# Frikallo/parakeet.cpp

Hardware: NVIDIA H100
Metric: audio-seconds/sec (RTFx) tdt-ctc-110m 10s clips (higher is better)
Workload: dtype bf16x3

## Files before the change

### parakeet.cpp_b200/csrc/attention_tc.cu

```cuda
#include "kernels.h"

namespace pk {
namespace {

constexpr int BQ = 64, BKV = 64;
constexpr int NPW = 128;
constexpr int LDG_ = 84;
constexpr int TCA_THREADS = 128;

template <int HD, bool QS>
struct __align__(16) AttnSmem {
    static constexpr int LDS_ = HD + 8;
    bf16 k_hi[BKV * LDS_], k_lo[BKV * LDS_];
    bf16 v_hi[BKV * LDS_], v_lo[BKV * LDS_];
    bf16 pp_hi[NPW * LDS_], pp_lo[NPW * LDS_];
    float g[QS ? 1 : 4][QS ? 4 : 16 * LDG_];
    bf16 q[QS ? 4 : 1][QS ? BQ * LDS_ : 8];
};
static_assert(sizeof(float) * 4 * 16 * LDG_ <= sizeof(bf16) * 2 * BKV * (128 + 8), "G patches must fit in the K tile");

__device__ __forceinline__ uint32_t smem_addr(const void *p) { return (uint32_t)__cvta_generic_to_shared(p); }
__device__ __forceinline__ void mma_bf16(float (&d)[4], const uint32_t (&a)[4], uint32_t b0, uint32_t b1) {
    asm volatile(
        "mma.sync.aligned.m16n8k16.row.col.f32.bf16.bf16.f32 {%0, %1, %2, %3}, {%4, %5, %6, %7}, {%8, %9}, {%0, %1, %2, %3};"
        : "+f"(d[0]), "+f"(d[1]), "+f"(d[2]), "+f"(d[3])
        : "r"(a[0]), "r"(a[1]), "r"(a[2]), "r"(a[3]), "r"(b0), "r"(b1));
}
__device__ __forceinline__ void ldsm_x4(uint32_t (&r)[4], uint32_t addr) {
    asm volatile("ldmatrix.sync.aligned.m8n8.x4.shared.b16 {%0, %1, %2, %3}, [%4];"
                 : "=r"(r[0]), "=r"(r[1]), "=r"(r[2]), "=r"(r[3]) : "r"(addr));
}
__device__ __forceinline__ void ldsm_x4_t(uint32_t (&r)[4], uint32_t addr) {
    asm volatile("ldmatrix.sync.aligned.m8n8.x4.trans.shared.b16 {%0, %1, %2, %3}, [%4];"
                 : "=r"(r[0]), "=r"(r[1]), "=r"(r[2]), "=r"(r[3]) : "r"(addr));
}
__device__ __forceinline__ void cp_async16(uint32_t dst, const void *src, int src_bytes) {
    asm volatile("cp.async.cg.shared.global [%0], [%1], 16, %2;" ::"r"(dst), "l"(src), "r"(src_bytes) : "memory");
}
__device__ __forceinline__ void split2(float x, float y, uint32_t &hi, uint32_t &lo) {
    __nv_bfloat162 h = __floats2bfloat162_rn(x, y);
    float2 hf = __bfloat1622float2(h);
    __nv_bfloat162 l = __floats2bfloat162_rn(x - hf.x, y - hf.y);
    hi = *reinterpret_cast<uint32_t *>(&h);
    lo = *reinterpret_cast<uint32_t *>(&l);
}
__device__ __forceinline__ float ex2_approx(float x) {
    float y;
    asm("ex2.approx.ftz.f32 %0, %1;" : "=f"(y) : "f"(x));
    return y;
}

template <int LDS_>
__device__ __forceinline__ uint32_t bfrag_addr(const bf16 *base, int n0, int k0, int lane) {
    return smem_addr(base + (n0 + ((lane >> 4) << 3) + (lane & 7)) * LDS_ + k0 + (((lane >> 3) & 1) << 3));
}
template <int LDS_>
__device__ __forceinline__ uint32_t afrag_addr(const bf16 *base, int m0, int k0, int lane) {
    return smem_addr(base + (m0 + (lane & 7) + (((lane >> 3) & 1) << 3)) * LDS_ + k0 + ((lane >> 4) << 3));
}
template <int LDS_>
__device__ __forceinline__ uint32_t bfrag_t_addr(const bf16 *base, int k0, int n0, int lane) {
    return smem_addr(base + (k0 + (((lane >> 3) & 1) << 3) + (lane & 7)) * LDS_ + n0 + ((lane >> 4) << 3));
}

template <int HD, bool QS>
__global__ void __launch_bounds__(TCA_THREADS, QS ? 1 : 2)
relpos_attention_tc_kernel(const float *__restrict__ q32, const float *__restrict__ pos_u, const float *__restrict__ pos_v,
                           const bf16 *__restrict__ qkv_hi, const bf16 *__restrict__ qkv_lo, int ld_qkv,
                           const int32_t *__restrict__ row_off, const bf16 *__restrict__ pp_hi,
                           const bf16 *__restrict__ pp_lo, int tmax, int d_model, ActBuf out) {
    pdl_wait();
    pdl_trigger();
    extern __shared__ __align__(16) uint8_t smraw[];
    using SM = AttnSmem<HD, QS>;
    constexpr int LDS_ = SM::LDS_, KS = HD / 16, NBO = HD / 8, CH = HD / 8;
    SM &sm = *reinterpret_cast<SM *>(smraw);
    const int b = blockIdx.z, h = blockIdx.y;
    const int r0 = row_off[b], T = row_off[b + 1] - r0;
    const int i0 = blockIdx.x * BQ;
    if (i0 >= T) return;
    const int tid = threadIdx.x, warp = tid >> 5, lane = tid & 31, g = lane >> 2, c = lane & 3;
    const int wrow = warp * 16;

    uint32_t qu_h[QS ? 1 : KS][4], qu_l[QS ? 1 : KS][4], qv_h[QS ? 1 : KS][4], qv_l[QS ? 1 : KS][4];
    constexpr int NQ = QS ? BQ * (HD / 4) / TCA_THREADS : 1;
    float4 qq[NQ];
    float2 qraw[QS ? 1 : KS][4];
    if (!QS) {
        const int ia = i0 + wrow + g, ib = ia + 8;
#pragma unroll
        for (int ks = 0; ks < (QS ? 1 : KS); ++ks)
#pragma unroll
            for (int e = 0; e < 4; ++e) {
                const int row = (e & 1) ? ib : ia;
                const int col = h * HD + ks * 16 + ((e >> 1) << 3) + 2 * c;
                qraw[ks][e] = make_float2(0.f, 0.f);
                if (row < T) qraw[ks][e] = *reinterpret_cast<const float2 *>(q32 + (size_t)(r0 + row) * d_model + col);
            }
    } else {
#pragma unroll
        for (int it = 0; it < NQ; ++it) {
            const int idx = tid + it * TCA_THREADS, i = idx / (HD / 4), c4 = (idx % (HD / 4)) * 4;
            qq[it] = make_float4(0.f, 0.f, 0.f, 0.f);
            if (i0 + i < T) qq[it] = *reinterpret_cast<const float4 *>(q32 + (size_t)(r0 + i0 + i) * d_model + h * HD + c4);
        }
    }

    float m_run[2] = {-INFINITY, -INFINITY}, l_run[2] = {0.f, 0.f};
    float oacc[NBO][4];
#pragma unroll
    for (int nb = 0; nb < NBO; ++nb)
#pragma unroll
        for (int e = 0; e < 4; ++e) oacc[nb][e] = 0.f;
    float *gs = QS ? reinterpret_cast<float *>(sm.k_hi) + warp * 16 * LDG_ : sm.g[QS ? 0 : warp];
    const uint32_t sk_hi = smem_addr(sm.k_hi), sk_lo = smem_addr(sm.k_lo), sv_hi = smem_addr(sm.v_hi), sv_lo = smem_addr(sm.v_lo);
    const uint32_t sp_hi = smem_addr(sm.pp_hi), sp_lo = smem_addr(sm.pp_lo);

    for (int j0 = 0; j0 < T; j0 += BKV) {
        __syncthreads();
        for (int idx = tid; idx < BKV * CH; idx += TCA_THREADS) {
            const int j = idx / CH, ch = idx % CH;
            const bool ok = (j0 + j < T);
            const size_t o = (size_t)(r0 + (ok ? j0 + j : 0)) * ld_qkv + h * HD + ch * 8;
            const uint32_t so = (uint32_t)(j * LDS_ + ch * 8) * 2u;
            const int nb = ok ? 16 : 0;
            cp_async16(sk_hi + so, qkv_hi + o, nb);
            cp_async16(sk_lo + so, qkv_lo + o, nb);
            cp_async16(sv_hi + so, qkv_hi + o + d_model, nb);
            cp_async16(sv_lo + so, qkv_lo + o + d_model, nb);
        }
        const int pmin = i0 - (j0 + BKV - 1);
        for (int idx = tid; idx < NPW * CH; idx += TCA_THREADS) {
            const int w = idx / CH, ch = idx % CH;
            const int prow = pmin + w + tmax - 1;
            const bool ok = (prow >= 0 && prow < 2 * tmax - 1);
            const size_t o = (size_t)(ok ? prow : 0) * d_model + h * HD + ch * 8;
            const uint32_t so = (uint32_t)(w * LDS_ + ch * 8) * 2u;
            const int nb = ok ? 16 : 0;
            cp_async16(sp_hi + so, pp_hi + o, nb);
            cp_async16(sp_lo + so, pp_lo + o, nb);
        }
        asm volatile("cp.async.commit_group;" ::: "memory");
        if (!QS && j0 == 0) {
            const int ia = i0 + wrow + g, ib = ia + 8;
#pragma unroll
            for (int ks = 0; ks < (QS ? 1 : KS); ++ks)
#pragma unroll
                for (int e = 0; e < 4; ++e) {
                    const int row = (e & 1) ? ib : ia;
                    const int col = h * HD + ks * 16 + ((e >> 1) << 3) + 2 * c;
                    const float2 bu = __ldg(reinterpret_cast<const float2 *>(pos_u + col)), bv = __ldg(reinterpret_cast<const float2 *>(pos_v + col));
                    const float2 qv2 = qraw[ks][e];
                    if (row < T) {
                        split2(qv2.x + bu.x, qv2.y + bu.y, qu_h[ks][e], qu_l[ks][e]);
                        split2(qv2.x + bv.x, qv2.y + bv.y, qv_h[ks][e], qv_l[ks][e]);
                    } else {
                        qu_h[ks][e] = qu_l[ks][e] = qv_h[ks][e] = qv_l[ks][e] = 0u;
                    }
                }
        }
        if (QS && j0 == 0) {
#pragma unroll
            for (int it = 0; it < NQ; ++it) {
                const int idx = tid + it * TCA_THREADS, i = idx / (HD / 4), c4 = (idx % (HD / 4)) * 4;
                const bool ok = (i0 + i < T);
                const float4 bu = __ldg(reinterpret_cast<const float4 *>(pos_u + h * HD + c4)), bv = __ldg(reinterpret_cast<const float4 *>(pos_v + h * HD + c4));
                uint2 uh = make_uint2(0u, 0u), ul = uh, vh = uh, vl = uh;
                if (ok) {
                    split2(qq[it].x + bu.x, qq[it].y + bu.y, uh.x, ul.x);
                    split2(qq[it].z + bu.z, qq[it].w + bu.w, uh.y, ul.y);
                    split2(qq[it].x + bv.x, qq[it].y + bv.y, vh.x, vl.x);
                    split2(qq[it].z + bv.z, qq[it].w + bv.w, vh.y, vl.y);
                }
                const int so = i * LDS_ + c4;
                *reinterpret_cast<uint2 *>(sm.q[0] + so) = uh;
                *reinterpret_cast<uint2 *>(sm.q[QS ? 1 : 0] + so) = ul;
                *reinterpret_cast<uint2 *>(sm.q[QS ? 2 : 0] + so) = vh;
                *reinterpret_cast<uint2 *>(sm.q[QS ? 3 : 0] + so) = vl;
            }
        }
        asm volatile("cp.async.wait_group 0;" ::: "memory");
        __syncthreads();

        float sacc[8][4];
#pragma unroll
        for (int nb = 0; nb < 8; ++nb)
#pragma unroll
            for (int e = 0; e < 4; ++e) sacc[nb][e] = 0.f;
#pragma unroll
        for (int ks = 0; ks < KS; ++ks) {
            uint32_t ah_[4], al_[4];
            if (QS) {
                ldsm_x4(ah_, afrag_addr<LDS_>(sm.q[0], wrow, ks * 16, lane));
                ldsm_x4(al_, afrag_addr<LDS_>(sm.q[QS ? 1 : 0], wrow, ks * 16, lane));
            }
            const uint32_t (&ah)[4] = QS ? ah_ : qu_h[QS ? 0 : ks];
            const uint32_t (&al)[4] = QS ? al_ : qu_l[QS ? 0 : ks];
#pragma unroll
            for (int np = 0; np < 4; ++np) {
                uint32_t bh[4], bl[4];
                ldsm_x4(bh, bfrag_addr<LDS_>(sm.k_hi, np * 16, ks * 16, lane));
                ldsm_x4(bl, bfrag_addr<LDS_>(sm.k_lo, np * 16, ks * 16, lane));
                mma_bf16(sacc[2 * np], ah, bh[0], bh[1]);
                mma_bf16(sacc[2 * np + 1], ah, bh[2], bh[3]);
                mma_bf16(sacc[2 * np], ah, bl[0], bl[1]);
                mma_bf16(sacc[2 * np + 1], ah, bl[2], bl[3]);
                mma_bf16(sacc[2 * np], al, bh[0], bh[1]);
                mma_bf16(sacc[2 * np + 1], al, bh[2], bh[3]);
            }
        }
        {
            float gacc[10][4];
#pragma unroll
            for (int nb = 0; nb < 10; ++nb)
#pragma unroll
                for (int e = 0; e < 4; ++e) gacc[nb][e] = 0.f;
#pragma unroll
            for (int ks = 0; ks < KS; ++ks) {
                uint32_t ah_[4], al_[4];
                if (QS) {
                    ldsm_x4(ah_, afrag_addr<LDS_>(sm.q[QS ? 2 : 0], wrow, ks * 16, lane));
                    ldsm_x4(al_, afrag_addr<LDS_>(sm.q[QS ? 3 : 0], wrow, ks * 16, lane));
                }
                const uint32_t (&ah)[4] = QS ? ah_ : qv_h[QS ? 0 : ks];
                const uint32_t (&al)[4] = QS ? al_ : qv_l[QS ? 0 : ks];
#pragma unroll
                for (int np = 0; np < 5; ++np) {
                    uint32_t bh[4], bl[4];
                    ldsm_x4(bh, bfrag_addr<LDS_>(sm.pp_hi, wrow + np * 16, ks * 16, lane));
                    ldsm_x4(bl, bfrag_addr<LDS_>(sm.pp_lo, wrow + np * 16, ks * 16, lane));
                    mma_bf16(gacc[2 * np], ah, bh[0], bh[1]);
                    mma_bf16(gacc[2 * np + 1], ah, bh[2], bh[3]);
                    mma_bf16(gacc[2 * np], ah, bl[0], bl[1]);
                    mma_bf16(gacc[2 * np + 1], ah, bl[2], bl[3]);
                    mma_bf16(gacc[2 * np], al, bh[0], bh[1]);
                    mma_bf16(gacc[2 * np + 1], al, bh[2], bh[3]);
                }
            }
            if (QS) __syncthreads();
#pragma unroll
            for (int nb = 0; nb < 10; ++nb) {
                *reinterpret_cast<float2 *>(gs + g * LDG_ + nb * 8 + 2 * c) = make_float2(gacc[nb][0], gacc[nb][1]);
                *reinterpret_cast<float2 *>(gs + (g + 8) * LDG_ + nb * 8 + 2 * c) = make_float2(gacc[nb][2], gacc[nb][3]);
            }
            __syncwarp();
#pragma unroll
            for (int nb = 0; nb < 8; ++nb)
#pragma unroll
                for (int e = 0; e < 2; ++e) {
                    const int jj = nb * 8 + 2 * c + e;
                    sacc[nb][e] += gs[g * LDG_ + g + (BKV - 1) - jj];
                    sacc[nb][2 + e] += gs[(g + 8) * LDG_ + g + 8 + (BKV - 1) - jj];
                }
            __syncwarp();
        }
        constexpr float kScale = (HD == 64 ? 0.125f : 0.08838834764831845f) * 1.4426950408889634f;
        static_assert(HD == 64 || HD == 128, "head_dim");
        float alpha[2];
#pragma unroll
        for (int hrow = 0; hrow < 2; ++hrow) {
            float mx = -INFINITY;
#pragma unroll
            for (int nb = 0; nb < 8; ++nb)
#pragma unroll
                for (int e = 0; e < 2; ++e) {
                    const int jj = nb * 8 + 2 * c + e;
                    float s = sacc[nb][hrow * 2 + e] * kScale;
                    s = (j0 + jj < T) ? s : -INFINITY;
                    sacc[nb][hrow * 2 + e] = s;
                    mx = fmaxf(mx, s);
                }
            mx = fmaxf(mx, __shfl_xor_sync(0xffffffffu, mx, 1));
            mx = fmaxf(mx, __shfl_xor_sync(0xffffffffu, mx, 2));
            const float m_new = fmaxf(m_run[hrow], mx);
            alpha[hrow] = ex2_approx(m_run[hrow] - m_new);
            float sum = 0.f;
#pragma unroll
            for (int nb = 0; nb < 8; ++nb)
#pragma unroll
                for (int e = 0; e < 2; ++e) {
                    const float pexp = ex2_approx(sacc[nb][hrow * 2 + e] - m_new);
                    sacc[nb][hrow * 2 + e] = pexp;
                    sum += pexp;
                }
            sum += __shfl_xor_sync(0xffffffffu, sum, 1);
            sum += __shfl_xor_sync(0xffffffffu, sum, 2);
            l_run[hrow] = l_run[hrow] * alpha[hrow] + sum;
            m_run[hrow] = m_new;
        }
#pragma unroll
        for (int nb = 0; nb < NBO; ++nb) {
            oacc[nb][0] *= alpha[0];
            oacc[nb][1] *= alpha[0];
            oacc[nb][2] *= alpha[1];
            oacc[nb][3] *= alpha[1];
        }
#pragma unroll
        for (int kk = 0; kk < BKV / 16; ++kk) {
            uint32_t ph[4], pl[4];
            split2(sacc[2 * kk][0], sacc[2 * kk][1], ph[0], pl[0]);
            split2(sacc[2 * kk][2], sacc[2 * kk][3], ph[1], pl[1]);
            split2(sacc[2 * kk + 1][0], sacc[2 * kk + 1][1], ph[2], pl[2]);
            split2(sacc[2 * kk + 1][2], sacc[2 * kk + 1][3], ph[3], pl[3]);
#pragma unroll
            for (int np = 0; np < HD / 16; ++np) {
                uint32_t bh[4], bl[4];
                ldsm_x4_t(bh, bfrag_t_addr<LDS_>(sm.v_hi, kk * 16, np * 16, lane));
                ldsm_x4_t(bl, bfrag_t_addr<LDS_>(sm.v_lo, kk * 16, np * 16, lane));
                mma_bf16(oacc[2 * np], ph, bh[0], bh[1]);
                mma_bf16(oacc[2 * np + 1], ph, bh[2], bh[3]);
                mma_bf16(oacc[2 * np], ph, bl[0], bl[1]);
                mma_bf16(oacc[2 * np + 1], ph, bl[2], bl[3]);
                mma_bf16(oacc[2 * np], pl, bh[0], bh[1]);
                mma_bf16(oacc[2 * np + 1], pl, bh[2], bh[3]);
            }
        }
    }
#pragma unroll
    for (int hrow = 0; hrow < 2; ++hrow) {
        const int i = i0 + wrow + g + hrow * 8;
        if (i >= T) continue;
        const float inv = 1.0f / l_run[hrow];
#pragma unroll
        for (int nb = 0; nb < NBO; ++nb) {
            const size_t idx = (size_t)(r0 + i) * d_model + h * HD + nb * 8 + 2 * c;
            const float x = oacc[nb][hrow * 2] * inv, y = oacc[nb][hrow * 2 + 1] * inv;
            if (out.f32) *reinterpret_cast<float2 *>(out.f32 + idx) = make_float2(x, y);
            if (out.hi) {
                uint32_t hi, lo;
                split2(x, y, hi, lo);
                *reinterpret_cast<uint32_t *>(out.hi + idx) = hi;
                if (out.lo) *reinterpret_cast<uint32_t *>(out.lo + idx) = lo;
            }
        }
    }
}

}

template <int HD, bool QS>
static bool launch_attn_t(const float *q32, const float *pos_u, const float *pos_v, const bf16 *qkv_hi, const bf16 *qkv_lo, int ld_qkv,
                          const int32_t *row_off, int n_utt, int max_T,
                          int n_heads, const bf16 *pp_hi, const bf16 *pp_lo, int tmax, int d_model, ActBuf out, cudaStream_t st) {
    using SM = AttnSmem<HD, QS>;
    static PerDeviceFlag attr_flag;
    bool &attr = attr_flag.cur();
    if (!attr) {
        if (cudaFuncSetAttribute(relpos_attention_tc_kernel<HD, QS>, cudaFuncAttributeMaxDynamicSharedMemorySize,
                                 (int)sizeof(SM)) != cudaSuccess)
            return false;
        attr = true;
    }
    dim3 grid((max_T + BQ - 1) / BQ, n_heads, n_utt);
    launch_pdl(relpos_attention_tc_kernel<HD, QS>, dim3(grid), dim3(TCA_THREADS), sizeof(SM), st, q32, pos_u, pos_v, qkv_hi, qkv_lo, ld_qkv, row_off, pp_hi, pp_lo,
                                                                              tmax, d_model, out);
    return true;
}

bool launch_relpos_attention_tc(const float *q32, const float *pos_u, const float *pos_v, const bf16 *qkv_hi, const bf16 *qkv_lo,
                                int ld_qkv, const int32_t *row_off, int n_utt, int max_T, int n_heads, int head_dim, const bf16 *pp_hi,
                                const bf16 *pp_lo, int tmax, int d_model, ActBuf out, cudaStream_t st) {
    if (!q32 || !pos_u || !pos_v || !qkv_hi || !qkv_lo || !pp_hi || !pp_lo) return false;
    if (head_dim == 64)
        return launch_attn_t<64, false>(q32, pos_u, pos_v, qkv_hi, qkv_lo, ld_qkv, row_off, n_utt, max_T, n_heads, pp_hi, pp_lo, tmax, d_model, out, st);
    if (head_dim == 128)
        return launch_attn_t<128, true>(q32, pos_u, pos_v, qkv_hi, qkv_lo, ld_qkv, row_off, n_utt, max_T, n_heads, pp_hi, pp_lo, tmax, d_model, out, st);
    return false;
}

}
```

Measured before the change: 44070.

## Make relpos attention persistent with double-buffered cp.async K/V/pos pipeline

Converts the relative-position attention kernel into a persistent grid that loops over (query block, head, utterance) items and prefetches the next item's data. K, V and positional tiles are staged through cp.async groups so loads overlap the QK, G and PV MMA stages. The positional window becomes a ring of 64-row slots reused across KV tiles instead of being reloaded as 128 rows each step. Q fragments are rebuilt from registers with the bias added on the fly, replacing the shared-memory Q staging. For head_dim 128 the block is now 8 warps with 128 query rows. This adds more synchronisation points and code complexity, and the persistent grid may balance poorly when there are few items.

```diff
diff --git a/parakeet.cpp_b200/csrc/attention_tc.cu b/parakeet.cpp_b200/csrc/attention_tc.cu
--- a/parakeet.cpp_b200/csrc/attention_tc.cu
+++ b/parakeet.cpp_b200/csrc/attention_tc.cu
@@ -3,21 +3,19 @@
 namespace pk {
 namespace {
 
-constexpr int BQ = 64, BKV = 64;
-constexpr int NPW = 128;
+constexpr int BKV = 64;
 constexpr int LDG_ = 84;
-constexpr int TCA_THREADS = 128;
-
-template <int HD, bool QS>
+
+template <int HD, int NW>
 struct __align__(16) AttnSmem {
-    static constexpr int LDS_ = HD + 8;
-    bf16 k_hi[BKV * LDS_], k_lo[BKV * LDS_];
-    bf16 v_hi[BKV * LDS_], v_lo[BKV * LDS_];
-    bf16 pp_hi[NPW * LDS_], pp_lo[NPW * LDS_];
-    float g[QS ? 1 : 4][QS ? 4 : 16 * LDG_];
-    bf16 q[QS ? 4 : 1][QS ? BQ * LDS_ : 8];
+    static constexpr int BQ = 16 * NW, NSLOT = NW / 4 + 1, LDS_ = HD + 8;
+    bf16 k[2][BKV * LDS_];
+    bf16 v[2][BKV * LDS_];
+    bf16 pp[NSLOT][2][BKV * LDS_];
+    float g[NW][16 * LDG_];
 };
-static_assert(sizeof(float) * 4 * 16 * LDG_ <= sizeof(bf16) * 2 * BKV * (128 + 8), "G patches must fit in the K tile");
+static_assert(sizeof(AttnSmem<128, 8>) <= 227 * 1024, "head_dim 128: one CTA per SM");
+static_assert(2 * (sizeof(AttnSmem<64, 4>) + 1024) <= 228 * 1024, "head_dim 64: two CTAs per SM");
 
 __device__ __forceinline__ uint32_t smem_addr(const void *p) { return (uint32_t)__cvta_generic_to_shared(p); }
 __device__ __forceinline__ void mma_bf16(float (&d)[4], const uint32_t (&a)[4], uint32_t b0, uint32_t b1) {
@@ -37,6 +35,8 @@
 __device__ __forceinline__ void cp_async16(uint32_t dst, const void *src, int src_bytes) {
     asm volatile("cp.async.cg.shared.global [%0], [%1], 16, %2;" ::"r"(dst), "l"(src), "r"(src_bytes) : "memory");
 }
+__device__ __forceinline__ void cp_async_commit() { asm volatile("cp.async.commit_group;" ::: "memory"); }
+__device__ __forceinline__ void cp_async_wait1() { asm volatile("cp.async.wait_group 1;" ::: "memory"); }
 __device__ __forceinline__ void split2(float x, float y, uint32_t &hi, uint32_t &lo) {
     __nv_bfloat162 h = __floats2bfloat162_rn(x, y);
     float2 hf = __bfloat1622float2(h);
@@ -51,199 +51,199 @@
 }
 
 template <int LDS_>
-__device__ __forceinline__ uint32_t bfrag_addr(const bf16 *base, int n0, int k0, int lane) {
-    return smem_addr(base + (n0 + ((lane >> 4) << 3) + (lane & 7)) * LDS_ + k0 + (((lane >> 3) & 1) << 3));
+__device__ __forceinline__ uint32_t bfrag_addr(uint32_t base, int n0, int k0, int lane) {
+    return base + 2u * (uint32_t)((n0 + ((lane >> 4) << 3) + (lane & 7)) * LDS_ + k0 + (((lane >> 3) & 1) << 3));
 }
 template <int LDS_>
-__device__ __forceinline__ uint32_t afrag_addr(const bf16 *base, int m0, int k0, int lane) {
-    return smem_addr(base + (m0 + (lane & 7) + (((lane >> 3) & 1) << 3)) * LDS_ + k0 + ((lane >> 4) << 3));
-}
-template <int LDS_>
-__device__ __forceinline__ uint32_t bfrag_t_addr(const bf16 *base, int k0, int n0, int lane) {
-    return smem_addr(base + (k0 + (((lane >> 3) & 1) << 3) + (lane & 7)) * LDS_ + n0 + ((lane >> 4) << 3));
-}
-
-template <int HD, bool QS>
-__global__ void __launch_bounds__(TCA_THREADS, QS ? 1 : 2)
+__device__ __forceinline__ uint32_t bfrag_t_addr(uint32_t base, int k0, int n0, int lane) {
+    return base + 2u * (uint32_t)((k0 + (((lane >> 3) & 1) << 3) + (lane & 7)) * LDS_ + n0 + ((lane >> 4) << 3));
+}
+
+template <int HD>
+__device__ __forceinline__ void qb_frag(const float2 (&q2)[4], const float *__restrict__ bias, int col0, bool oka, bool okb,
+                                        uint32_t (&hi)[4], uint32_t (&lo)[4]) {
+#pragma unroll
+    for (int e = 0; e < 4; ++e) {
+        const float2 bb = __ldg(reinterpret_cast<const float2 *>(bias + col0 + ((e >> 1) << 3)));
+        if ((e & 1) ? okb : oka) {
+            split2(q2[e].x + bb.x, q2[e].y + bb.y, hi[e], lo[e]);
+        } else {
+            hi[e] = lo[e] = 0u;
+        }
+    }
+}
+
+template <int HD, int NW>
+__global__ void __launch_bounds__(32 * NW, NW == 4 ? 2 : 1)
 relpos_attention_tc_kernel(const float *__restrict__ q32, const float *__restrict__ pos_u, const float *__restrict__ pos_v,
                            const bf16 *__restrict__ qkv_hi, const bf16 *__restrict__ qkv_lo, int ld_qkv,
                            const int32_t *__restrict__ row_off, const bf16 *__restrict__ pp_hi,
-                           const bf16 *__restrict__ pp_lo, int tmax, int d_model, ActBuf out) {
+                           const bf16 *__restrict__ pp_lo, int tmax, int d_model, int n_qb, int n_heads, int n_items, ActBuf out) {
     pdl_wait();
     pdl_trigger();
     extern __shared__ __align__(16) uint8_t smraw[];
-    using SM = AttnSmem<HD, QS>;
+    using SM = AttnSmem<HD, NW>;
+    constexpr int BQ = SM::BQ, NSLOT = SM::NSLOT, NTHR = 32 * NW;
     constexpr int LDS_ = SM::LDS_, KS = HD / 16, NBO = HD / 8, CH = HD / 8;
+    constexpr uint32_t PLANE = BKV * LDS_ * 2u;
     SM &sm = *reinterpret_cast<SM *>(smraw);
-    const int b = blockIdx.z, h = blockIdx.y;
-    const int r0 = row_off[b], T = row_off[b + 1] - r0;
-    const int i0 = blockIdx.x * BQ;
-    if (i0 >= T) return;
     const int tid = threadIdx.x, warp = tid >> 5, lane = tid & 31, g = lane >> 2, c = lane & 3;
     const int wrow = warp * 16;
-
-    uint32_t qu_h[QS ? 1 : KS][4], qu_l[QS ? 1 : KS][4], qv_h[QS ? 1 : KS][4], qv_l[QS ? 1 : KS][4];
-    constexpr int NQ = QS ? BQ * (HD / 4) / TCA_THREADS : 1;
-    float4 qq[NQ];
-    float2 qraw[QS ? 1 : KS][4];
-    if (!QS) {
-        const int ia = i0 + wrow + g, ib = ia + 8;
-#pragma unroll
-        for (int ks = 0; ks < (QS ? 1 : KS); ++ks)
+    const uint32_t sk = smem_addr(sm.k[0]), sv = smem_addr(sm.v[0]), sp = smem_addr(sm.pp[0][0]);
+
+    struct Item { int it, h, i0, r0, T; };
+    auto decode = [&](int it) {
+        Item x;
+        x.it = it;
+        x.i0 = (it % n_qb) * BQ;
+        x.h = (it / n_qb) % n_heads;
+        const int b = it / (n_qb * n_heads);
+        x.r0 = row_off[b];
+        x.T = row_off[b + 1] - x.r0;
+        return x;
+    };
+    auto next_item = [&](int it) {
+        for (; it < n_items; it += gridDim.x)
+            if (decode(it).i0 < decode(it).T) return it;
+        return n_items;
+    };
+    auto copy_kv = [&](uint32_t dst, const Item &x, int j0, int plane_off) {
+        for (int idx = tid; idx < BKV * CH; idx += NTHR) {
+            const int j = idx / CH, ch = idx % CH;
+            const bool ok = (j0 + j < x.T);
+            const size_t o = (size_t)(x.r0 + (ok ? j0 + j : 0)) * ld_qkv + plane_off + x.h * HD + ch * 8;
+            const uint32_t so = (uint32_t)(j * LDS_ + ch * 8) * 2u;
+            const int nb = ok ? 16 : 0;
+            cp_async16(dst + so, qkv_hi + o, nb);
+            cp_async16(dst + PLANE + so, qkv_lo + o, nb);
+        }
+    };
+    auto copy_pp = [&](int slot, const Item &x, int m) {
+        const uint32_t dst = sp + (uint32_t)slot * 2u * PLANE;
+        const int p0 = x.i0 + tmax + BKV * (NSLOT - 2) - BKV * m;
+        for (int idx = tid; idx < BKV * CH; idx += NTHR) {
+            const int w = idx / CH, ch = idx % CH;
+            const int prow = p0 + w;
+            const bool ok = (prow >= 0 && prow < 2 * tmax - 1);
+            const size_t o = (size_t)(ok ? prow : 0) * d_model + x.h * HD + ch * 8;
+            const uint32_t so = (uint32_t)(w * LDS_ + ch * 8) * 2u;
+            const int nb = ok ? 16 : 0;
+            cp_async16(dst + so, pp_hi + o, nb);
+            cp_async16(dst + PLANE + so, pp_lo + o, nb);
+        }
+    };
+    float2 qraw[KS][4];
+    auto load_q = [&](const Item &x) {
+        const int ia = x.i0 + wrow + g, ib = ia + 8;
+#pragma unroll
+        for (int ks = 0; ks < KS; ++ks)
 #pragma unroll
             for (int e = 0; e < 4; ++e) {
                 const int row = (e & 1) ? ib : ia;
-                const int col = h * HD + ks * 16 + ((e >> 1) << 3) + 2 * c;
+                const int col = x.h * HD + ks * 16 + ((e >> 1) << 3) + 2 * c;
                 qraw[ks][e] = make_float2(0.f, 0.f);
-                if (row < T) qraw[ks][e] = *reinterpret_cast<const float2 *>(q32 + (size_t)(r0 + row) * d_model + col);
-            }
-    } else {
-#pragma unroll
-        for (int it = 0; it < NQ; ++it) {
-            const int idx = tid + it * TCA_THREADS, i = idx / (HD / 4), c4 = (idx % (HD / 4)) * 4;
-            qq[it] = make_float4(0.f, 0.f, 0.f, 0.f);
-            if (i0 + i < T) qq[it] = *reinterpret_cast<const float4 *>(q32 + (size_t)(r0 + i0 + i) * d_model + h * HD + c4);
-        }
-    }
-
-    float m_run[2] = {-INFINITY, -INFINITY}, l_run[2] = {0.f, 0.f};
-    float oacc[NBO][4];
-#pragma unroll
-    for (int nb = 0; nb < NBO; ++nb)
-#pragma unroll
-        for (int e = 0; e < 4; ++e) oacc[nb][e] = 0.f;
-    float *gs = QS ? reinterpret_cast<float *>(sm.k_hi) + warp * 16 * LDG_ : sm.g[QS ? 0 : warp];
-    const uint32_t sk_hi = smem_addr(sm.k_hi), sk_lo = smem_addr(sm.k_lo), sv_hi = smem_addr(sm.v_hi), sv_lo = smem_addr(sm.v_lo);
-    const uint32_t sp_hi = smem_addr(sm.pp_hi), sp_lo = smem_addr(sm.pp_lo);
-
-    for (int j0 = 0; j0 < T; j0 += BKV) {
-        __syncthreads();
-        for (int idx = tid; idx < BKV * CH; idx += TCA_THREADS) {
-            const int j = idx / CH, ch = idx % CH;
-            const bool ok = (j0 + j < T);
-            const size_t o = (size_t)(r0 + (ok ? j0 + j : 0)) * ld_qkv + h * HD + ch * 8;
-            const uint32_t so = (uint32_t)(j * LDS_ + ch * 8) * 2u;
-            const int nb = ok ? 16 : 0;
-            cp_async16(sk_hi + so, qkv_hi + o, nb);
-            cp_async16(sk_lo + so, qkv_lo + o, nb);
-            cp_async16(sv_hi + so, qkv_hi + o + d_model, nb);
-            cp_async16(sv_lo + so, qkv_lo + o + d_model, nb);
-        }
-        const int pmin = i0 - (j0 + BKV - 1);
-        for (int idx = tid; idx < NPW * CH; idx += TCA_THREADS) {
-            const int w = idx / CH, ch = idx % CH;
-            const int prow = pmin + w + tmax - 1;
-            const bool ok = (prow >= 0 && prow < 2 * tmax - 1);
-            const size_t o = (size_t)(ok ? prow : 0) * d_model + h * HD + ch * 8;
-            const uint32_t so = (uint32_t)(w * LDS_ + ch * 8) * 2u;
-            const int nb = ok ? 16 : 0;
-            cp_async16(sp_hi + so, pp_hi + o, nb);
-            cp_async16(sp_lo + so, pp_lo + o, nb);
-        }
-        asm volatile("cp.async.commit_group;" ::: "memory");
-        if (!QS && j0 == 0) {
-            const int ia = i0 + wrow + g, ib = ia + 8;
-#pragma unroll
-            for (int ks = 0; ks < (QS ? 1 : KS); ++ks)
-#pragma unroll
-                for (int e = 0; e < 4; ++e) {
-                    const int row = (e & 1) ? ib : ia;
-                    const int col = h * HD + ks * 16 + ((e >> 1) << 3) + 2 * c;
-                    const float2 bu = __ldg(reinterpret_cast<const float2 *>(pos_u + col)), bv = __ldg(reinterpret_cast<const float2 *>(pos_v + col));
-                    const float2 qv2 = qraw[ks][e];
-                    if (row < T) {
-                        split2(qv2.x + bu.x, qv2.y + bu.y, qu_h[ks][e], qu_l[ks][e]);
-                        split2(qv2.x + bv.x, qv2.y + bv.y, qv_h[ks][e], qv_l[ks][e]);
-                    } else {
-                        qu_h[ks][e] = qu_l[ks][e] = qv_h[ks][e] = qv_l[ks][e] = 0u;
+                if (row < x.T) qraw[ks][e] = *reinterpret_cast<const float2 *>(q32 + (size_t)(x.r0 + row) * d_model + col);
+            }
+    };
+
+    const int it0 = next_item(blockIdx.x);
+    if (it0 >= n_items) return;
+    Item cur = decode(it0);
+    load_q(cur);
+    for (int m = 0; m < NSLOT; ++m) copy_pp(m, cur, m);
+    cp_async_commit();
+    copy_kv(sk, cur, 0, 0);
+    cp_async_commit();
+    int cb = 0;
+
+    while (true) {
+        const int h = cur.h, i0 = cur.i0, r0 = cur.r0, T = cur.T;
+        const int ntile = (T + BKV - 1) / BKV;
+        const int ia = i0 + wrow + g, ib = ia + 8;
+        const bool oka = ia < T, okb = ib < T;
+        const int nxt_it = next_item(cur.it + gridDim.x);
+        const bool has_next = nxt_it < n_items;
+
+        float m_run[2] = {-INFINITY, -INFINITY}, l_run[2] = {0.f, 0.f};
+        float oacc[NBO][4];
+#pragma unroll
+        for (int nb = 0; nb < NBO; ++nb)
+#pragma unroll
+            for (int e = 0; e < 4; ++e) oacc[nb][e] = 0.f;
+        float *gs = sm.g[warp];
+
+        for (int t = 0; t < ntile; ++t) {
+            const int j0 = t * BKV;
+            cp_async_wait1();
+            __syncthreads();
+            copy_kv(sv, cur, j0, d_model);
+            cp_async_commit();
+
+            {
+                float gacc[10][4];
+#pragma unroll
+                for (int nb = 0; nb < 10; ++nb)
+#pragma unroll
+                    for (int e = 0; e < 4; ++e) gacc[nb][e] = 0.f;
+#pragma unroll
+                for (int ks = 0; ks < KS; ++ks) {
+                    uint32_t ah[4], al[4];
+                    qb_frag<HD>(qraw[ks], pos_v, h * HD + ks * 16 + 2 * c, oka, okb, ah, al);
+#pragma unroll
+                    for (int np = 0; np < 5; ++np) {
+                        const int w0 = wrow + np * 16;
+                        const uint32_t base = sp + (uint32_t)((cb + t + NSLOT - 1 - w0 / BKV) % NSLOT) * 2u * PLANE;
+                        const uint32_t a = bfrag_addr<LDS_>(base, w0 & (BKV - 1), ks * 16, lane);
+                        uint32_t bh[4], bl[4];
+                        ldsm_x4(bh, a);
+                        ldsm_x4(bl, a + PLANE);
+                        mma_bf16(gacc[2 * np], ah, bh[0], bh[1]);
+                        mma_bf16(gacc[2 * np + 1], ah, bh[2], bh[3]);
+                        mma_bf16(gacc[2 * np], ah, bl[0], bl[1]);
+                        mma_bf16(gacc[2 * np + 1], ah, bl[2], bl[3]);
+                        mma_bf16(gacc[2 * np], al, bh[0], bh[1]);
+                        mma_bf16(gacc[2 * np + 1], al, bh[2], bh[3]);
                     }
                 }
-        }
-        if (QS && j0 == 0) {
-#pragma unroll
-            for (int it = 0; it < NQ; ++it) {
-                const int idx = tid + it * TCA_THREADS, i = idx / (HD / 4), c4 = (idx % (HD / 4)) * 4;
-                const bool ok = (i0 + i < T);
-                const float4 bu = __ldg(reinterpret_cast<const float4 *>(pos_u + h * HD + c4)), bv = __ldg(reinterpret_cast<const float4 *>(pos_v + h * HD + c4));
-                uint2 uh = make_uint2(0u, 0u), ul = uh, vh = uh, vl = uh;
-                if (ok) {
-                    split2(qq[it].x + bu.x, qq[it].y + bu.y, uh.x, ul.x);
-                    split2(qq[it].z + bu.z, qq[it].w + bu.w, uh.y, ul.y);
-                    split2(qq[it].x + bv.x, qq[it].y + bv.y, vh.x, vl.x);
-                    split2(qq[it].z + bv.z, qq[it].w + bv.w, vh.y, vl.y);
-                }
-                const int so = i * LDS_ + c4;
-                *reinterpret_cast<uint2 *>(sm.q[0] + so) = uh;
-                *reinterpret_cast<uint2 *>(sm.q[QS ? 1 : 0] + so) = ul;
-                *reinterpret_cast<uint2 *>(sm.q[QS ? 2 : 0] + so) = vh;
-                *reinterpret_cast<uint2 *>(sm.q[QS ? 3 : 0] + so) = vl;
-            }
-        }
-        asm volatile("cp.async.wait_group 0;" ::: "memory");
-        __syncthreads();
-
-        float sacc[8][4];
-#pragma unroll
-        for (int nb = 0; nb < 8; ++nb)
-#pragma unroll
-            for (int e = 0; e < 4; ++e) sacc[nb][e] = 0.f;
-#pragma unroll
-        for (int ks = 0; ks < KS; ++ks) {
-            uint32_t ah_[4], al_[4];
-            if (QS) {
-                ldsm_x4(ah_, afrag_addr<LDS_>(sm.q[0], wrow, ks * 16, lane));
-                ldsm_x4(al_, afrag_addr<LDS_>(sm.q[QS ? 1 : 0], wrow, ks * 16, lane));
-            }
-            const uint32_t (&ah)[4] = QS ? ah_ : qu_h[QS ? 0 : ks];
-            const uint32_t (&al)[4] = QS ? al_ : qu_l[QS ? 0 : ks];
-#pragma unroll
-            for (int np = 0; np < 4; ++np) {
-                uint32_t bh[4], bl[4];
-                ldsm_x4(bh, bfrag_addr<LDS_>(sm.k_hi, np * 16, ks * 16, lane));
-                ldsm_x4(bl, bfrag_addr<LDS_>(sm.k_lo, np * 16, ks * 16, lane));
-                mma_bf16(sacc[2 * np], ah, bh[0], bh[1]);
-                mma_bf16(sacc[2 * np + 1], ah, bh[2], bh[3]);
-                mma_bf16(sacc[2 * np], ah, bl[0], bl[1]);
-                mma_bf16(sacc[2 * np + 1], ah, bl[2], bl[3]);
-                mma_bf16(sacc[2 * np], al, bh[0], bh[1]);
-                mma_bf16(sacc[2 * np + 1], al, bh[2], bh[3]);
-            }
-        }
-        {
-            float gacc[10][4];
-#pragma unroll
-            for (int nb = 0; nb < 10; ++nb)
-#pragma unroll
-                for (int e = 0; e < 4; ++e) gacc[nb][e] = 0.f;
+#pragma unroll
+                for (int nb = 0; nb < 10; ++nb) {
+                    *reinterpret_cast<float2 *>(gs + g * LDG_ + nb * 8 + 2 * c) = make_float2(gacc[nb][0], gacc[nb][1]);
+                    *reinterpret_cast<float2 *>(gs + (g + 8) * LDG_ + nb * 8 + 2 * c) = make_float2(gacc[nb][2], gacc[nb][3]);
+                }
+            }
+
+            cp_async_wait1();
+            __syncthreads();
+            if (t + 1 < ntile) {
+                copy_pp((cb + t + NSLOT) % NSLOT, cur, t + NSLOT);
+            } else if (has_next) {
+#pragma unroll
+                for (int m = 0; m < NSLOT; ++m) copy_pp((cb + ntile + NSLOT - 1 + m) % NSLOT, decode(nxt_it), m);
+            }
+            cp_async_commit();
+            float sacc[8][4];
+#pragma unroll
+            for (int nb = 0; nb < 8; ++nb)
+#pragma unroll
+                for (int e = 0; e < 4; ++e) sacc[nb][e] = 0.f;
 #pragma unroll
             for (int ks = 0; ks < KS; ++ks) {
-                uint32_t ah_[4], al_[4];
-                if (QS) {
-                    ldsm_x4(ah_, afrag_addr<LDS_>(sm.q[QS ? 2 : 0], wrow, ks * 16, lane));
-                    ldsm_x4(al_, afrag_addr<LDS_>(sm.q[QS ? 3 : 0], wrow, ks * 16, lane));
-                }
-                const uint32_t (&ah)[4] = QS ? ah_ : qv_h[QS ? 0 : ks];
-                const uint32_t (&al)[4] = QS ? al_ : qv_l[QS ? 0 : ks];
-#pragma unroll
-                for (int np = 0; np < 5; ++np) {
+                uint32_t ah[4], al[4];
+                qb_frag<HD>(qraw[ks], pos_u, h * HD + ks * 16 + 2 * c, oka, okb, ah, al);
+#pragma unroll
+                for (int np = 0; np < 4; ++np) {
+                    const uint32_t a = bfrag_addr<LDS_>(sk, np * 16, ks * 16, lane);
                     uint32_t bh[4], bl[4];
-                    ldsm_x4(bh, bfrag_addr<LDS_>(sm.pp_hi, wrow + np * 16, ks * 16, lane));
-                    ldsm_x4(bl, bfrag_addr<LDS_>(sm.pp_lo, wrow + np * 16, ks * 16, lane));
-                    mma_bf16(gacc[2 * np], ah, bh[0], bh[1]);
-                    mma_bf16(gacc[2 * np + 1], ah, bh[2], bh[3]);
-                    mma_bf16(gacc[2 * np], ah, bl[0], bl[1]);
-                    mma_bf16(gacc[2 * np + 1], ah, bl[2], bl[3]);
-                    mma_bf16(gacc[2 * np], al, bh[0], bh[1]);
-                    mma_bf16(gacc[2 * np + 1], al, bh[2], bh[3]);
-                }
-            }
-            if (QS) __syncthreads();
-#pragma unroll
-            for (int nb = 0; nb < 10; ++nb) {
-                *reinterpret_cast<float2 *>(gs + g * LDG_ + nb * 8 + 2 * c) = make_float2(gacc[nb][0], gacc[nb][1]);
-                *reinterpret_cast<float2 *>(gs + (g + 8) * LDG_ + nb * 8 + 2 * c) = make_float2(gacc[nb][2], gacc[nb][3]);
-            }
-            __syncwarp();
+                    ldsm_x4(bh, a);
+                    ldsm_x4(bl, a + PLANE);
+                    mma_bf16(sacc[2 * np], ah, bh[0], bh[1]);
+                    mma_bf16(sacc[2 * np + 1], ah, bh[2], bh[3]);
+                    mma_bf16(sacc[2 * np], ah, bl[0], bl[1]);
+                    mma_bf16(sacc[2 * np + 1], ah, bl[2], bl[3]);
+                    mma_bf16(sacc[2 * np], al, bh[0], bh[1]);
+                    mma_bf16(sacc[2 * np + 1], al, bh[2], bh[3]);
+                }
+            }
 #pragma unroll
             for (int nb = 0; nb < 8; ++nb)
 #pragma unroll
@@ -252,108 +252,131 @@
                     sacc[nb][e] += gs[g * LDG_ + g + (BKV - 1) - jj];
                     sacc[nb][2 + e] += gs[(g + 8) * LDG_ + g + 8 + (BKV - 1) - jj];
                 }
-            __syncwarp();
-        }
-        constexpr float kScale = (HD == 64 ? 0.125f : 0.08838834764831845f) * 1.4426950408889634f;
-        static_assert(HD == 64 || HD == 128, "head_dim");
-        float alpha[2];
+            constexpr float kScale = (HD == 64 ? 0.125f : 0.08838834764831845f) * 1.4426950408889634f;
+            static_assert(HD == 64 || HD == 128, "head_dim");
+            float alpha[2];
+#pragma unroll
+            for (int hrow = 0; hrow < 2; ++hrow) {
+                float mx = -INFINITY;
+#pragma unroll
+                for (int nb = 0; nb < 8; ++nb)
+#pragma unroll
+                    for (int e = 0; e < 2; ++e) {
+                        const int jj = nb * 8 + 2 * c + e;
+                        float s = sacc[nb][hrow * 2 + e] * kScale;
+                        s = (j0 + jj < T) ? s : -INFINITY;
+                        sacc[nb][hrow * 2 + e] = s;
+                        mx = fmaxf(mx, s);
+                    }
+                mx = fmaxf(mx, __shfl_xor_sync(0xffffffffu, mx, 1));
+                mx = fmaxf(mx, __shfl_xor_sync(0xffffffffu, mx, 2));
+                const float m_new = fmaxf(m_run[hrow], mx);
+                alpha[hrow] = ex2_approx(m_run[hrow] - m_new);
+                float sum = 0.f;
+#pragma unroll
+                for (int nb = 0; nb < 8; ++nb)
+#pragma unroll
+                    for (int e = 0; e < 2; ++e) {
+                        const float pexp = ex2_approx(sacc[nb][hrow * 2 + e] - m_new);
+                        sacc[nb][hrow * 2 + e] = pexp;
+                        sum += pexp;
+                    }
+                sum += __shfl_xor_sync(0xffffffffu, sum, 1);
+                sum += __shfl_xor_sync(0xffffffffu, sum, 2);
+                l_run[hrow] = l_run[hrow] * alpha[hrow] + sum;
+                m_run[hrow] = m_new;
+            }
+#pragma unroll
+            for (int nb = 0; nb < NBO; ++nb) {
+                oacc[nb][0] *= alpha[0];
+                oacc[nb][1] *= alpha[0];
+                oacc[nb][2] *= alpha[1];
+                oacc[nb][3] *= alpha[1];
+            }
+
+            cp_async_wait1();
+            __syncthreads();
+            if (t + 1 < ntile) {
+                copy_kv(sk, cur, j0 + BKV, 0);
+            } else if (has_next) {
+                copy_kv(sk, decode(nxt_it), 0, 0);
+            }
+            cp_async_commit();
+
+#pragma unroll
+            for (int kk = 0; kk < BKV / 16; ++kk) {
+                uint32_t ph[4], pl[4];
+                split2(sacc[2 * kk][0], sacc[2 * kk][1], ph[0], pl[0]);
+                split2(sacc[2 * kk][2], sacc[2 * kk][3], ph[1], pl[1]);
+                split2(sacc[2 * kk + 1][0], sacc[2 * kk + 1][1], ph[2], pl[2]);
+                split2(sacc[2 * kk + 1][2], sacc[2 * kk + 1][3], ph[3], pl[3]);
+#pragma unroll
+                for (int np = 0; np < HD / 16; ++np) {
+                    const uint32_t a = bfrag_t_addr<LDS_>(sv, kk * 16, np * 16, lane);
+                    uint32_t bh[4], bl[4];
+                    ldsm_x4_t(bh, a);
+                    ldsm_x4_t(bl, a + PLANE);
+                    mma_bf16(oacc[2 * np], ph, bh[0], bh[1]);
+                    mma_bf16(oacc[2 * np + 1], ph, bh[2], bh[3]);
+                    mma_bf16(oacc[2 * np], ph, bl[0], bl[1]);
+                    mma_bf16(oacc[2 * np + 1], ph, bl[2], bl[3]);
+                    mma_bf16(oacc[2 * np], pl, bh[0], bh[1]);
+                    mma_bf16(oacc[2 * np + 1], pl, bh[2], bh[3]);
+                }
+            }
+        }
+        if (has_next) load_q(decode(nxt_it));
 #pragma unroll
         for (int hrow = 0; hrow < 2; ++hrow) {
-            float mx = -INFINITY;
-#pragma unroll
-            for (int nb = 0; nb < 8; ++nb)
-#pragma unroll
-                for (int e = 0; e < 2; ++e) {
-                    const int jj = nb * 8 + 2 * c + e;
-                    float s = sacc[nb][hrow * 2 + e] * kScale;
-                    s = (j0 + jj < T) ? s : -INFINITY;
-                    sacc[nb][hrow * 2 + e] = s;
-                    mx = fmaxf(mx, s);
-                }
-            mx = fmaxf(mx, __shfl_xor_sync(0xffffffffu, mx, 1));
-            mx = fmaxf(mx, __shfl_xor_sync(0xffffffffu, mx, 2));
-            const float m_new = fmaxf(m_run[hrow], mx);
-            alpha[hrow] = ex2_approx(m_run[hrow] - m_new);
-            float sum = 0.f;
-#pragma unroll
-            for (int nb = 0; nb < 8; ++nb)
-#pragma unroll
-                for (int e = 0; e < 2; ++e) {
-                    const float pexp = ex2_approx(sacc[nb][hrow * 2 + e] - m_new);
-                    sacc[nb][hrow * 2 + e] = pexp;
-                    sum += pexp;
-                }
-            sum += __shfl_xor_sync(0xffffffffu, sum, 1);
-            sum += __shfl_xor_sync(0xffffffffu, sum, 2);
-            l_run[hrow] = l_run[hrow] * alpha[hrow] + sum;
-            m_run[hrow] = m_new;
-        }
-#pragma unroll
-        for (int nb = 0; nb < NBO; ++nb) {
-            oacc[nb][0] *= alpha[0];
-            oacc[nb][1] *= alpha[0];
-            oacc[nb][2] *= alpha[1];
-            oacc[nb][3] *= alpha[1];
-        }
-#pragma unroll
-        for (int kk = 0; kk < BKV / 16; ++kk) {
-            uint32_t ph[4], pl[4];
-            split2(sacc[2 * kk][0], sacc[2 * kk][1], ph[0], pl[0]);
-            split2(sacc[2 * kk][2], sacc[2 * kk][3], ph[1], pl[1]);
-            split2(sacc[2 * kk + 1][0], sacc[2 * kk + 1][1], ph[2], pl[2]);
-            split2(sacc[2 * kk + 1][2], sacc[2 * kk + 1][3], ph[3], pl[3]);
-#pragma unroll
-            for (int np = 0; np < HD / 16; ++np) {
-                uint32_t bh[4], bl[4];
-                ldsm_x4_t(bh, bfrag_t_addr<LDS_>(sm.v_hi, kk * 16, np * 16, lane));
-                ldsm_x4_t(bl, bfrag_t_addr<LDS_>(sm.v_lo, kk * 16, np * 16, lane));
-                mma_bf16(oacc[2 * np], ph, bh[0], bh[1]);
-                mma_bf16(oacc[2 * np + 1], ph, bh[2], bh[3]);
-                mma_bf16(oacc[2 * np], ph, bl[0], bl[1]);
-                mma_bf16(oacc[2 * np + 1], ph, bl[2], bl[3]);
-                mma_bf16(oacc[2 * np], pl, bh[0], bh[1]);
-                mma_bf16(oacc[2 * np + 1], pl, bh[2], bh[3]);
-            }
-        }
+            const int i = i0 + wrow + g + hrow * 8;
+            if (i >= T) continue;
+            const float inv = 1.0f / l_run[hrow];
+#pragma unroll
+            for (int nb = 0; nb < NBO; ++nb) {
+                const size_t idx = (size_t)(r0 + i) * d_model + h * HD + nb * 8 + 2 * c;
+                const float x = oacc[nb][hrow * 2] * inv, y = oacc[nb][hrow * 2 + 1] * inv;
+                if (out.f32) *reinterpret_cast<float2 *>(out.f32 + idx) = make_float2(x, y);
+                if (out.hi) {
+                    uint32_t hi, lo;
+                    split2(x, y, hi, lo);
+                    *reinterpret_cast<uint32_t *>(out.hi + idx) = hi;
+                    if (out.lo) *reinterpret_cast<uint32_t *>(out.lo + idx) = lo;
+                }
+            }
+        }
+        if (!has_next) break;
+        cb += ntile + NSLOT - 1;
+        cur = decode(nxt_it);
     }
-#pragma unroll
-    for (int hrow = 0; hrow < 2; ++hrow) {
-        const int i = i0 + wrow + g + hrow * 8;
-        if (i >= T) continue;
-        const float inv = 1.0f / l_run[hrow];
-#pragma unroll
-        for (int nb = 0; nb < NBO; ++nb) {
-            const size_t idx = (size_t)(r0 + i) * d_model + h * HD + nb * 8 + 2 * c;
-            const float x = oacc[nb][hrow * 2] * inv, y = oacc[nb][hrow * 2 + 1] * inv;
-            if (out.f32) *reinterpret_cast<float2 *>(out.f32 + idx) = make_float2(x, y);
-            if (out.hi) {
-                uint32_t hi, lo;
-                split2(x, y, hi, lo);
-                *reinterpret_cast<uint32_t *>(out.hi + idx) = hi;
-                if (out.lo) *reinterpret_cast<uint32_t *>(out.lo + idx) = lo;
-            }
-        }
-    }
-}
-
-}
-
-template <int HD, bool QS>
+}
+
+}
+
+template <int HD, int NW>
 static bool launch_attn_t(const float *q32, const float *pos_u, const float *pos_v, const bf16 *qkv_hi, const bf16 *qkv_lo, int ld_qkv,
                           const int32_t *row_off, int n_utt, int max_T,
                           int n_heads, const bf16 *pp_hi, const bf16 *pp_lo, int tmax, int d_model, ActBuf out, cudaStream_t st) {
-    using SM = AttnSmem<HD, QS>;
+    using SM = AttnSmem<HD, NW>;
     static PerDeviceFlag attr_flag;
     bool &attr = attr_flag.cur();
     if (!attr) {
-        if (cudaFuncSetAttribute(relpos_attention_tc_kernel<HD, QS>, cudaFuncAttributeMaxDynamicSharedMemorySize,
+        if (cudaFuncSetAttribute(relpos_attention_tc_kernel<HD, NW>, cudaFuncAttributeMaxDynamicSharedMemorySize,
                                  (int)sizeof(SM)) != cudaSuccess)
             return false;
         attr = true;
     }
-    dim3 grid((max_T + BQ - 1) / BQ, n_heads, n_utt);
-    launch_pdl(relpos_attention_tc_kernel<HD, QS>, dim3(grid), dim3(TCA_THREADS), sizeof(SM), st, q32, pos_u, pos_v, qkv_hi, qkv_lo, ld_qkv, row_off, pp_hi, pp_lo,
-                                                                              tmax, d_model, out);
+    static PerDeviceFlag sms_flag;
+    size_t &sms = sms_flag.cur_size();
+    if (!sms) {
+        int dev = 0, v = 0;
+        if (cudaGetDevice(&dev) != cudaSuccess || cudaDeviceGetAttribute(&v, cudaDevAttrMultiProcessorCount, dev) != cudaSuccess || v < 1)
+            return false;
+        sms = (size_t)v;
+    }
+    const int n_qb = (max_T + SM::BQ - 1) / SM::BQ, n_items = n_qb * n_heads * n_utt;
+    const int ctas = (int)std::min<size_t>((size_t)n_items, sms * (NW == 4 ? 2 : 1));
+    launch_pdl(relpos_attention_tc_kernel<HD, NW>, dim3(ctas), dim3(32 * NW), sizeof(SM), st, q32, pos_u, pos_v, qkv_hi, qkv_lo, ld_qkv, row_off, pp_hi, pp_lo,
+               tmax, d_model, n_qb, n_heads, n_items, out);
     return true;
 }
 
@@ -362,9 +385,9 @@
                                 const bf16 *pp_lo, int tmax, int d_model, ActBuf out, cudaStream_t st) {
     if (!q32 || !pos_u || !pos_v || !qkv_hi || !qkv_lo || !pp_hi || !pp_lo) return false;
     if (head_dim == 64)
-        return launch_attn_t<64, false>(q32, pos_u, pos_v, qkv_hi, qkv_lo, ld_qkv, row_off, n_utt, max_T, n_heads, pp_hi, pp_lo, tmax, d_model, out, st);
+        return launch_attn_t<64, 4>(q32, pos_u, pos_v, qkv_hi, qkv_lo, ld_qkv, row_off, n_utt, max_T, n_heads, pp_hi, pp_lo, tmax, d_model, out, st);
     if (head_dim == 128)
-        return launch_attn_t<128, true>(q32, pos_u, pos_v, qkv_hi, qkv_lo, ld_qkv, row_off, n_utt, max_T, n_heads, pp_hi, pp_lo, tmax, d_model, out, st);
+        return launch_attn_t<128, 8>(q32, pos_u, pos_v, qkv_hi, qkv_lo, ld_qkv, row_off, n_utt, max_T, n_heads, pp_hi, pp_lo, tmax, d_model, out, st);
     return false;
 }
 
```

New measurement: 44170 (median of 6 runs). Within noise of the previous version (+0.2%).
